# jonassibbesen/rpvg

Measured on AMD Instinct MI355X. Metric: read-pairs quantified/sec, higher is better.
Workload: dtype f64

## Files before the change

rpvg_amd/csrc/bounded_search.hip:

```cpp

#include "common.hpp"

#include <algorithm>
#include <cstdlib>
#include <map>
#include <memory>
#include <mutex>
#include <numeric>

using namespace rpvg_hip_detail;

namespace {
std::mutex g_search_gate_mutex;
const rpvg_hip_ctx * g_search_gate_owner = nullptr;
}

static bool searchLaunchesEarly() {
    static const bool early = RPVG_EXPERIMENT_ENV("RPVG_HIP_SEARCH_LAUNCH_EARLY") != nullptr;
    return early;
}

constexpr uint64_t kSearchGateRows = 1ull << 17;

static void searchGateEnter(rpvg_hip_ctx * ctx, hipStream_t stream, const uint64_t matrix_rows) {
    static const bool open_gate = RPVG_EXPERIMENT_ENV("RPVG_HIP_NO_SEARCH_GATE") != nullptr;
    ctx->search_gate_held = !open_gate && matrix_rows >= kSearchGateRows;
    if (!ctx->search_gate_held) return;
    hipEvent_t previous = nullptr;
    {
        std::lock_guard<std::mutex> lock(g_search_gate_mutex);
        if (g_search_gate_owner && g_search_gate_owner != ctx && g_search_gate_owner->device == ctx->device) {
            previous = g_search_gate_owner->search_done;
            (void) hipStreamWaitEvent(stream, previous, 0);
        }
    }
    if (previous && !searchLaunchesEarly()) (void) waitEvent(previous);
}

static void searchGateLeave(rpvg_hip_ctx * ctx, hipStream_t stream) {
    if (!ctx->search_gate_held) return;
    ctx->search_gate_held = false;
    std::lock_guard<std::mutex> lock(g_search_gate_mutex);
    (void) hipEventRecord(ctx->search_done, stream);
    g_search_gate_owner = ctx;
}

void searchGateForget(const rpvg_hip_ctx * ctx) {
    std::lock_guard<std::mutex> lock(g_search_gate_mutex);
    if (g_search_gate_owner == ctx) g_search_gate_owner = nullptr;
}

struct rpvg_hip_pair_posteriors {
    std::vector<uint64_t> pair_off;
    void * block = nullptr;
    bool block_pinned = false;
    const uint32_t * first = nullptr, * second = nullptr;
    const double * posterior = nullptr;
    ~rpvg_hip_pair_posteriors() {
        if (block && block_pinned) pinnedFree(block);
        else std::free(block);
    }
};

namespace {

constexpr uint32_t kLdsRows = 2048;
constexpr uint32_t kSmallRows = 512;
constexpr uint32_t kSmallRowLdsCols = 128;
constexpr uint32_t kRowLdsCols = 512;

__device__ __forceinline__ double waveSum(double v) { return waveSumF64(v); }

__device__ __forceinline__ double addLog(const double log_x, const double log_y) {
    return log_x > log_y ? log_x + log1p(exp(log_y - log_x)) : log_y + log1p(exp(log_x - log_y));
}


template <int kBlock, typename ValueFn>
__device__ __forceinline__ double blockLogSumExp(const uint32_t n, ValueFn value, double * scratch) {
    const double lowest = -1.7976931348623157e308;
    const int lane = threadIdx.x & 63, wave = threadIdx.x >> 6;
    double mx = lowest;
    for (uint32_t k = threadIdx.x; k < n; k += kBlock) mx = fmax(mx, value(k));
#pragma unroll
    for (int d = 32; d >= 1; d >>= 1) mx = fmax(mx, __shfl_xor(mx, d, 64));
    __syncthreads();
    if (lane == 0) scratch[wave] = mx;
    __syncthreads();
#pragma unroll
    for (int w2 = 0; w2 < kBlock / 64; ++w2) mx = fmax(mx, scratch[w2]);
    double sum = 0.0;
    for (uint32_t k = threadIdx.x; k < n; k += kBlock) {
        const double v = value(k);
        if (v > lowest) sum += exp(v - mx);
    }
    sum = waveSum(sum);
    __syncthreads();
    if (lane == 0) scratch[wave] = sum;
    __syncthreads();
    double total = 0.0;
#pragma unroll
    for (int w2 = 0; w2 < kBlock / 64; ++w2) total += scratch[w2];
    return (n == 0 || !(mx > lowest)) ? lowest : mx + log(total);
}

struct SearchArgs {
    const uint32_t * order;
    uint32_t count;
    const uint64_t * mat_val_off;
    const uint64_t * mat_row_off;
    const uint32_t * mat_fast;
    const uint32_t * mat_mid;
    const uint64_t * mat_rows;
    const uint32_t * mat_cols;
    const double * values;
    const double * rowmax;
    const double * row_count;
    const double * row_noise;
    const uint64_t * col_off;
    const uint32_t * col_count;
    const uint64_t * pair_cap_off;
    double min_log_likelihood_diff;
    uint32_t stage_rows;
    uint32_t row_lds_cols;
    double * log_freq;
    double * marginal;
    double * optimistic_raw;
    double * optimistic;
    uint32_t * col_order;
    uint32_t * out_first;
    uint32_t * out_second;
    double * out_value;
    uint32_t * out_count;
    unsigned long long * log_evals;
};

constexpr int kTileFirst = 4;

template <int kGroup>
__device__ __forceinline__ void tilePairSums(const LogTableEntry * lt, const double * lds_count, const double * lds_base, const uint32_t stride,
                                             const double * __restrict__ cnt, const double * __restrict__ nz,
                                             const double * const (&col_a)[kTileFirst], const double * __restrict__ col_b, const uint32_t staged,
                                             const uint64_t fast_end, const uint64_t mid_end, const uint64_t R, const int lane,
                                             double (&out)[kTileFirst]) {
    LogProduct pr[kTileFirst];
    double acc[kTileFirst];
#pragma unroll
    for (int t = 0; t < kTileFirst; ++t) acc[t] = 0.0;
    auto clip = [&](const uint64_t v) { return static_cast<uint32_t>(v < staged ? v : staged); };
    sumCountLogsMulti<kTileFirst, kGroup, uint32_t>(lt, lds_count, [&](const uint32_t i, double (&xs)[kTileFirst]) {
        const double x = col_b[i] / 2.0;
#pragma unroll
        for (int t = 0; t < kTileFirst; ++t) xs[t] = lds_base[t * stride + i] + x;
    }, 0u, clip(fast_end), clip(mid_end), staged, lane, pr, acc);
    if (staged < R) {
        sumCountLogsMulti<kTileFirst, kGroup, uint64_t>(lt, cnt, [&](const uint64_t i, double (&xs)[kTileFirst]) {
            const double noise = nz[i], x = col_b[i] / 2.0;
#pragma unroll
            for (int t = 0; t < kTileFirst; ++t) xs[t] = (noise + col_a[t][i] / 2.0) + x;
        }, static_cast<uint64_t>(staged), fast_end, mid_end, R, lane, pr, acc);
    }
#pragma unroll
    for (int t = 0; t < kTileFirst; ++t) out[t] = mid_end ? acc[t] + pr[t].value(lt) : acc[t];
}

template <int kBlock, int kGroup>
__global__ __launch_bounds__(kBlock) __attribute__((amdgpu_waves_per_eu(4))) void boundedSearchKernel(const SearchArgs args) {
    constexpr int kWaves = kBlock / 64;
    constexpr int kGroupsPerWave = 64 / kGroup;
    extern __shared__ __attribute__((aligned(16))) double lds_dyn[];
    double * lds_base = lds_dyn;
    double * lds_count = lds_dyn + kTileFirst * args.stage_rows;
    double * lds_rows = lds_count + args.stage_rows;
    __shared__ double lds_red[kBlock / 64];
    __shared__ unsigned long long lds_sum;
    __shared__ LogTableEntry lt[kLogTableSize];

    if (blockIdx.x >= args.count) return;
    loadLogTable(lt);
    const uint32_t m = args.order[blockIdx.x];
    const int lane = threadIdx.x & 63, wave = threadIdx.x >> 6;
    const uint64_t R = args.mat_rows[m];
    const uint32_t G = args.mat_cols[m];
    const double * M = args.values + args.mat_val_off[m];
    const double * rm = args.rowmax + args.mat_row_off[m];
    const double * cnt = args.row_count + args.mat_row_off[m];
    const double * nz = args.row_noise + args.mat_row_off[m];
    const uint64_t fast_end = args.mat_fast[m], mid_end = args.mat_mid[m];
    const uint64_t c0 = args.col_off[m];
    const uint32_t * ccount = args.col_count + c0;
    double * lf = args.log_freq + c0;
    double * marg = args.marginal + c0;
    double * opt_raw = args.optimistic_raw + c0;
    double * opt = args.optimistic + c0;
    uint32_t * ord = args.col_order + c0;
    const uint64_t p0 = args.pair_cap_off[m];
    uint32_t * out_first = args.out_first + p0;
    uint32_t * out_second = args.out_second + p0;
    double * out_value = args.out_value + p0;
    const double thr = args.min_log_likelihood_diff;
    const double lowest = -1.7976931348623157e308;
    const double log_two = log(2.0);

    if (threadIdx.x == 0) lds_sum = 0;
    __syncthreads();
    unsigned long long part = 0;
    for (uint32_t g = threadIdx.x; g < G; g += kBlock) part += ccount[g];
    if (part) atomicAdd(&lds_sum, part);
    __syncthreads();
    const double count_sum = static_cast<double>(lds_sum);
    for (uint32_t g = threadIdx.x; g < G; g += kBlock) lf[g] = log(ccount[g] / count_sum);
    __syncthreads();

    for (uint32_t g = wave; g < G; g += kWaves) {
        const double * col = M + static_cast<uint64_t>(g) * R;
        double acc1 = sumCountLogs<uint64_t>(lt, cnt, [&](const uint64_t i) { return nz[i] + col[i] / 1.0; }, 0, fast_end, mid_end, R, lane);
        double acc2 = sumCountLogs<uint64_t>(lt, cnt, [&](const uint64_t i) { return (nz[i] + col[i] / 2.0) + rm[i] / 2.0; }, 0, fast_end, mid_end, R, lane);
        acc1 = waveSum(acc1);
        acc2 = waveSum(acc2);
        if (lane == 0) {
            marg[g] = (acc1 + lf[g]) + 0.0;
            opt_raw[g] = acc2 + (lf[g] + log_two);
        }
    }
    __syncthreads();

    {
        const double sum_log = blockLogSumExp<kBlock>(G, [&](uint32_t g) { return marg[g]; }, lds_red);
        for (uint32_t g = threadIdx.x; g < G; g += kBlock) marg[g] = exp(marg[g] - sum_log);
    }
    __syncthreads();

    for (uint32_t g = threadIdx.x; g < G; g += kBlock) {
        const double pg = marg[g];
        uint32_t rank = 0;
        for (uint32_t h = 0; h < G; ++h) {
            const double ph = marg[h];
            rank += (ph > pg || (ph == pg && h > g)) ? 1u : 0u;
        }
        ord[rank] = g;
        opt[rank] = opt_raw[g];
    }
    __syncthreads();

    const bool rows_in_lds = G <= args.row_lds_cols;
    const uint32_t tile_max = rows_in_lds ? kTileFirst : 1;
    const uint32_t row_stride = rows_in_lds ? args.row_lds_cols : 0;
    double * row_ll = rows_in_lds ? lds_rows : opt_raw;
    const uint32_t stride = args.stage_rows;

    double max_ll = lowest;
    uint32_t kept = 0;
    unsigned long long pairs_evaluated = 0;
    const uint32_t staged = static_cast<uint32_t>(R < args.stage_rows ? R : args.stage_rows);
    uint32_t pos = 0;
    while (pos < G) {
        uint32_t tile_pos[kTileFirst];
        uint32_t nt = 0;
        while (pos < G && nt < tile_max) {
            if (!(opt[pos] - max_ll < thr)) tile_pos[nt++] = pos;
            ++pos;
        }
        if (nt == 0) break;
#pragma unroll
        for (int t = 1; t < kTileFirst; ++t)
            if (t >= static_cast<int>(nt)) tile_pos[t] = tile_pos[0];
        uint32_t a[kTileFirst];
        const double * col_a[kTileFirst];
#pragma unroll
        for (int t = 0; t < kTileFirst; ++t) {
            a[t] = ord[tile_pos[t]];
            col_a[t] = M + static_cast<uint64_t>(a[t]) * R;
        }
        __syncthreads();
        for (uint32_t i = threadIdx.x; i < staged; i += kBlock) {
            const double noise = nz[i];
#pragma unroll
            for (int t = 0; t < kTileFirst; ++t) lds_base[t * stride + i] = noise + col_a[t][i] / 2.0;
            lds_count[i] = cnt[i];
        }
        __syncthreads();
        for (uint32_t t = 0; t < nt; ++t) pairs_evaluated += G - tile_pos[t];
        const uint32_t j0 = tile_pos[0];
        const int sub = lane & (kGroup - 1), grp = lane / kGroup;
        for (uint32_t jw = j0 + wave * kGroupsPerWave; jw < G; jw += kWaves * kGroupsPerWave) {
            const uint32_t j = jw + grp;
            const bool valid = j < G;
            const uint32_t b = ord[valid ? j : G - 1];
            double sums[kTileFirst];
            tilePairSums<kGroup>(lt, lds_count, lds_base, stride, cnt, nz, col_a, M + static_cast<uint64_t>(b) * R, staged, fast_end, mid_end, R, sub, sums);
            const double lf_b = lf[b];
#pragma unroll
            for (int t = 0; t < kTileFirst; ++t) {
                const double total = kGroup == 64 ? waveSum(sums[t]) : rowSumF64(sums[t]);
                if (sub == 0 && valid && t < static_cast<int>(nt) && j >= tile_pos[t]) {
                    row_ll[t * row_stride + (j - tile_pos[t])] = total + ((lf[a[t]] + lf_b) + (a[t] == b ? 0.0 : log_two));
                }
            }
        }
        __syncthreads();
        for (uint32_t t = 0; t < nt; ++t) {
            if (t > 0 && opt[tile_pos[t]] - max_ll < thr) continue;
            const double * row = row_ll + t * row_stride;
            const uint32_t n = G - tile_pos[t];
            if (thr <= 0.0) {
                for (uint32_t c = 0; c < n; c += 64) {
                    const uint32_t k = c + lane;
                    const double ll = k < n ? row[k] : lowest;
                    double incl = ll;
#pragma unroll
                    for (int d = 1; d < 64; d <<= 1) {
                        const double up = __shfl_up(incl, d, 64);
                        if (lane >= d) incl = fmax(incl, up);
                    }
                    double before = __shfl_up(incl, 1, 64);
                    before = lane == 0 ? max_ll : fmax(max_ll, before);
                    const bool keep = k < n && !(ll - before < thr);
                    const unsigned long long ballot = __ballot(keep);
                    if (keep && wave == 0) {
                        const uint32_t slot = kept + __popcll(ballot & ((1ull << lane) - 1ull));
                        out_first[slot] = a[t];
                        out_second[slot] = ord[tile_pos[t] + k];
                        out_value[slot] = ll;
                    }
                    kept += __popcll(ballot);
                    max_ll = fmax(max_ll, __shfl(incl, 63, 64));
                }
            } else {
                for (uint32_t k = 0; k < n; ++k) {
                    const double ll = row[k];
                    if (!(ll - max_ll < thr)) {
                        max_ll = fmax(max_ll, ll);
                        if (threadIdx.x == 0) {
                            out_first[kept] = a[t];
                            out_second[kept] = ord[tile_pos[t] + k];
                            out_value[kept] = ll;
                        }
                        ++kept;
                    }
                }
            }
        }
    }

    __syncthreads();
    if (threadIdx.x == 0) {
        args.out_count[m] = kept;
        atomicAdd(args.log_evals, (2ull * G + pairs_evaluated) * R);
    }
    {
        auto kept_value = [&](uint32_t k) { const double ll = out_value[k]; return (ll - max_ll < thr) ? lowest : ll; };
        const double sum_log = blockLogSumExp<kBlock>(kept, kept_value, lds_red);
        for (uint32_t k = threadIdx.x; k < kept; k += kBlock) out_value[k] = exp(kept_value(k) - sum_log);
    }
}



constexpr uint32_t kChunkRows = 1024;
constexpr int kTileA = 4;

struct TableWork {
    const uint32_t * item_matrix;
    const uint32_t * item_col;
    const uint32_t * item_chunk;
    uint32_t count;
    const uint64_t * mat_val_off;
    const uint64_t * mat_row_off;
    const uint32_t * mat_fast;
    const uint32_t * mat_mid;
    const uint64_t * mat_rows;
    const uint32_t * mat_cols;
    const double * values;
    const double * rowmax;
    const double * row_count;
    const double * row_noise;
    const uint64_t * big_col_part_off;
    const uint64_t * big_pair_part_off;
    double * part_marginal;
    double * part_optimistic;
    double * part_pair;
    unsigned long long * log_evals;
};

__global__ __launch_bounds__(256) void pairTableKernel(const TableWork w) {
    __shared__ double lds_base[kTileA][kChunkRows];
    __shared__ double lds_count[kChunkRows];
    __shared__ LogTableEntry lt[kLogTableSize];
    const uint32_t per_xcd = (w.count + 7) / 8;
    const uint32_t item = (blockIdx.x % 8) * per_xcd + blockIdx.x / 8;
    if (item >= w.count) return;
    loadLogTable(lt);
    const uint32_t m = w.item_matrix[item], a0 = w.item_col[item], chunk = w.item_chunk[item];
    const int lane = threadIdx.x & 63, wave = threadIdx.x >> 6;
    const uint64_t R = w.mat_rows[m];
    const uint32_t G = w.mat_cols[m];
    const uint32_t ta = (G - a0) < kTileA ? (G - a0) : kTileA;
    const uint64_t r_begin = static_cast<uint64_t>(chunk) * kChunkRows;
    const uint32_t n = static_cast<uint32_t>((R - r_begin) < kChunkRows ? (R - r_begin) : kChunkRows);
    const double * M = w.values + w.mat_val_off[m] + r_begin;
    const double * cnt = w.row_count + w.mat_row_off[m] + r_begin;
    const double * nz = w.row_noise + w.mat_row_off[m] + r_begin;
    auto local = [&](const uint64_t end_row) { return end_row <= r_begin ? 0u : (end_row - r_begin < n ? static_cast<uint32_t>(end_row - r_begin) : n); };
    const uint32_t nf = local(w.mat_fast[m]), nm = local(w.mat_mid[m]);

    for (uint32_t i = threadIdx.x; i < n; i += 256) {
        const double noise = nz[i];
        lds_count[i] = cnt[i];
#pragma unroll
        for (int t = 0; t < kTileA; ++t) {
            const uint32_t a = a0 + (t < static_cast<int>(ta) ? t : 0);
            lds_base[t][i] = noise + M[static_cast<uint64_t>(a) * R + i] / 2.0;
        }
    }
    __syncthreads();
    const uint32_t num_tasks = ta + (G - a0);
    for (uint32_t task = wave; task < num_tasks; task += 4) {
        if (task < ta) {
            const uint32_t a = a0 + task;
            const double * col_a = M + static_cast<uint64_t>(a) * R;
            const double acc = waveSum(sumCountLogs<uint32_t>(lt, lds_count, [&](const uint32_t i) { return nz[i] + col_a[i] / 1.0; }, 0u, nf, nm, n, lane));
            if (lane == 0) w.part_marginal[w.big_col_part_off[m] + static_cast<uint64_t>(chunk) * G + a] = acc;
        } else {
            const uint32_t b = a0 + (task - ta);
            const double * col_b = M + static_cast<uint64_t>(b) * R;
            double acc[kTileA];
            LogProduct pr[kTileA];
#pragma unroll
            for (int t = 0; t < kTileA; ++t) acc[t] = 0.0;
            sumCountLogsMulti<kTileA, 64, uint32_t>(lt, lds_count, [&](const uint32_t i, double (&xs)[kTileA]) {
                const double x = col_b[i] / 2.0;
#pragma unroll
                for (int t = 0; t < kTileA; ++t) xs[t] = lds_base[t][i] + x;
            }, 0u, nf, nm, n, lane, pr, acc);
            if (nm) {
#pragma unroll
                for (int t = 0; t < kTileA; ++t) acc[t] += pr[t].value(lt);
            }
#pragma unroll
            for (int t = 0; t < kTileA; ++t) {
                const double total = waveSum(acc[t]);
                if (lane == 0 && t < static_cast<int>(ta) && a0 + t <= b) {
                    w.part_pair[w.big_pair_part_off[m] + (static_cast<uint64_t>(chunk) * G + (a0 + t)) * G + b] = total;
                }
            }
        }
    }
    if (threadIdx.x == 0) atomicAdd(w.log_evals, static_cast<unsigned long long>(ta + (G - a0) * kTileA) * n);
}


constexpr uint32_t kTileBlock = 256;
constexpr uint32_t kTileLdsDoubles = 6 * 1024;
constexpr uint32_t kTileMaxColumns = 1024;

__host__ __device__ inline uint32_t tileColumns(const uint32_t G) { return (G + 3) / 4; }
__host__ __device__ inline uint32_t tileCount(const uint32_t G) { return tileColumns(G) * (tileColumns(G) + 1) / 2; }
__host__ __device__ inline uint32_t tileSlices(const uint32_t G) { return tileCount(G) <= kTileBlock ? kTileBlock / tileCount(G) : 1u; }
__host__ __device__ inline uint32_t marginalSlices(const uint32_t G) { return kTileBlock / tileColumns(G); }

struct PairTileWork {
    const uint32_t * item_matrix;
    const uint32_t * item_chunk;
    const uint32_t * item_tiles;
    uint32_t chunk_rows;
    uint32_t count;
    const uint64_t * mat_val_off;
    const uint64_t * mat_row_off;
    const uint32_t * mat_fast;
    const uint32_t * mat_mid;
    const uint64_t * mat_rows;
    const uint32_t * mat_cols;
    const double * values;
    const double * row_count;
    const double * row_noise;
    const uint64_t * col_part_off;
    const uint64_t * pair_part_off;
    double * part_marginal;
    double * part_pair;
    unsigned long long * log_evals;
#ifdef RPVG_HIP_EXPERIMENTS
    uint32_t debug_skip;
#endif
};

#ifdef RPVG_HIP_EXPERIMENTS
#define RPVG_PAIR_DEBUG_SKIP(w) ((w).debug_skip)
#else
#define RPVG_PAIR_DEBUG_SKIP(w) 0u
#endif

constexpr uint32_t kTile2BufferDoubles = 3 * 1024;

__host__ __device__ inline uint32_t tileRowOfTile(const uint32_t t, const uint32_t T) {
    uint32_t lo = 0, hi = T - 1;
    while (lo < hi) {
        const uint32_t mid = (lo + hi + 1) >> 1;
        if (mid * T - mid * (mid - 1) / 2 <= t) lo = mid; else hi = mid - 1;
    }
    return lo;
}

__device__ __forceinline__ void ldsDirectLoad16(const double * from, double * lds_wave_base) {
    __builtin_amdgcn_global_load_lds((const __attribute__((address_space(1))) void *)from, (__attribute__((address_space(3))) void *)lds_wave_base, 16, 0, 0);
}

template <uint32_t kSubRows>
__device__ __forceinline__ void ldsReadRow(const uint32_t noise_at, const uint32_t u_at, const uint32_t v_at, double & noise, double (&u)[4], double (&v)[4]) {
    asm volatile("ds_read_b64 %0, %9\n\t"
                 "ds_read_b64 %1, %10\n\t"
                 "ds_read_b64 %2, %10 offset:%12\n\t"
                 "ds_read_b64 %3, %10 offset:%13\n\t"
                 "ds_read_b64 %4, %10 offset:%14\n\t"
                 "ds_read_b64 %5, %11\n\t"
                 "ds_read_b64 %6, %11 offset:%12\n\t"
                 "ds_read_b64 %7, %11 offset:%13\n\t"
                 "ds_read_b64 %8, %11 offset:%14"
                 : "=&v"(noise), "=&v"(u[0]), "=&v"(u[1]), "=&v"(u[2]), "=&v"(u[3]), "=&v"(v[0]), "=&v"(v[1]), "=&v"(v[2]), "=&v"(v[3])
                 : "v"(noise_at), "v"(u_at), "v"(v_at), "i"(kSubRows * 8), "i"(kSubRows * 16), "i"(kSubRows * 24));
}

__device__ __forceinline__ void ldsRowLanded(double & noise, double (&u)[4], double (&v)[4]) {
    asm volatile("s_waitcnt lgkmcnt(0)" : "+v"(noise), "+v"(u[0]), "+v"(u[1]), "+v"(u[2]), "+v"(u[3]), "+v"(v[0]), "+v"(v[1]), "+v"(v[2]), "+v"(v[3]));
}

__device__ __forceinline__ uint32_t ldsByteAddress(const double * const p) {
    return static_cast<uint32_t>(reinterpret_cast<uintptr_t>(p));
}

__host__ __device__ inline uint32_t tileSubRows(const uint32_t ncols) {
    const uint32_t fit = (kTile2BufferDoubles - ncols / 2) / (ncols + 2);
    return fit >= 126 ? 126u : fit >= 94 ? 94u : fit >= 46 ? 46u : fit >= 30 ? 30u : fit >= 14 ? 14u : fit >= 6 ? 6u : 2u;
}

template <uint32_t kSubRows>
__device__ __forceinline__ void pairTile2Item(const PairTileWork & w, double * const tile_lds, const LogTableEntry * const lt, const uint32_t m, const uint32_t chunk,
                                              const uint32_t t0, const uint32_t tcount, const uint32_t c_lo, const uint32_t ncols) {
    const uint64_t R = w.mat_rows[m];
    const uint32_t G = w.mat_cols[m];
    const uint32_t T = tileColumns(G);
    const uint32_t S = kTileBlock / tcount;
    constexpr uint32_t sub_rows = kSubRows;
    const uint32_t lanes_per_column = sub_rows / 2, columns_per_load = lanes_per_column <= 16 ? 4u : lanes_per_column <= 32 ? 2u : 1u;
    auto columnOffset = [&](const uint32_t c) { return static_cast<size_t>(c) * sub_rows + (c / 4) * 2; };
    const uint64_t r_begin = static_cast<uint64_t>(chunk) * w.chunk_rows;
    const uint32_t n = static_cast<uint32_t>((R - r_begin) < w.chunk_rows ? (R - r_begin) : w.chunk_rows);
    const double * M = w.values + w.mat_val_off[m] + r_begin;
    const double * cnt = w.row_count + w.mat_row_off[m] + r_begin;
    const double * nz = w.row_noise + w.mat_row_off[m] + r_begin;
    auto local = [&](const uint64_t end_row) { return end_row <= r_begin ? 0u : (end_row - r_begin < n ? static_cast<uint32_t>(end_row - r_begin) : n); };
    const uint32_t nf = local(w.mat_fast[m]), nm = local(w.mat_mid[m]);
    const uint32_t lane = threadIdx.x & 63u, wave = threadIdx.x >> 6;

    const uint32_t buffer_doubles = (ncols + 2) * sub_rows + ncols / 2;
    auto stage = [&](const uint32_t s0, const uint32_t ns, double * const buffer) {
        if (RPVG_PAIR_DEBUG_SKIP(w) & 16u) return;
        const uint32_t pairs = (ns + 1) / 2;
        const uint32_t col_in_load = lane / lanes_per_column, pair = lane % lanes_per_column;
        const bool lane_loads = col_in_load < columns_per_load && pair < pairs;
        for (uint32_t c0 = wave * columns_per_load; c0 < ncols; c0 += 4 * columns_per_load) {
            const uint32_t c = c0 + col_in_load;
            if (lane_loads && c < ncols) {
                const uint32_t column = c_lo + c < G ? c_lo + c : G - 1;
                ldsDirectLoad16(M + static_cast<uint64_t>(column) * R + s0 + 2 * pair, buffer + columnOffset(c0));
            }
        }
        if (wave < 2 && lane < pairs) {
            ldsDirectLoad16((wave == 0 ? nz : cnt) + s0 + 2 * lane, buffer + columnOffset(ncols) + wave * sub_rows);
        }
    };

    const uint32_t t = t0 + threadIdx.x % tcount, slice = threadIdx.x / tcount;
    const bool active = slice < S;
    const uint32_t ta = tileRowOfTile(t, T);
    const uint32_t tb = ta + (t - (ta * T - ta * (ta > 0 ? ta - 1 : 0) / 2));
    const uint32_t SM = marginalSlices(G);
    const uint32_t tc = threadIdx.x % T, marg_slice = threadIdx.x / T;
    const bool with_marginals = t0 == 0 && marg_slice < SM && !(RPVG_PAIR_DEBUG_SKIP(w) & 8u);

    LogProduct pr[4][4], prm[4];
    double acc[4][4], accm[4];
#pragma unroll
    for (int i = 0; i < 4; ++i) {
        accm[i] = 0.0;
#pragma unroll
        for (int j = 0; j < 4; ++j) acc[i][j] = 0.0;
    }
    uint32_t since_fold = 0, since_fold_m = 0;
    int doubled = 0;
    auto foldPairs = [&]() {
#pragma unroll
        for (int i = 0; i < 4; ++i) {
#pragma unroll
            for (int j = 0; j < 4; ++j) pr[i][j].fold();
        }
        since_fold = 0;
    };
    auto foldMarginals = [&]() {
#pragma unroll
        for (int i = 0; i < 4; ++i) prm[i].fold();
        since_fold_m = 0;
    };

    const uint32_t blocks = (n + sub_rows - 1) / sub_rows;
    if (RPVG_PAIR_DEBUG_SKIP(w) & 64u) return;
    if (RPVG_PAIR_DEBUG_SKIP(w) & 16u) {
        for (uint32_t i = threadIdx.x; i < 2 * kTile2BufferDoubles; i += kTileBlock) tile_lds[i] = 0.25;
    }
    stage(0, n < sub_rows ? n : sub_rows, tile_lds);
    for (uint32_t blk = 0; blk < blocks; ++blk) {
        const uint32_t s0 = blk * sub_rows;
        const uint32_t ns = (n - s0) < sub_rows ? (n - s0) : sub_rows;
        double * const H = tile_lds + static_cast<size_t>(blk & 1u) * buffer_doubles;
        asm volatile("s_waitcnt vmcnt(0)" ::: "memory");
        __syncthreads();
        if (blk + 1 < blocks) {
            const uint32_t s1 = s0 + sub_rows;
            stage(s1, (n - s1) < sub_rows ? (n - s1) : sub_rows, tile_lds + static_cast<size_t>((blk + 1) & 1u) * buffer_doubles);
        }
        const double * const lds_noise = H + columnOffset(ncols);
        const double * const lds_count = lds_noise + sub_rows;
        const uint32_t f1 = nf <= s0 ? 0u : ((nf - s0) < ns ? (nf - s0) : ns);
        const uint32_t m1 = nm <= s0 ? 0u : ((nm - s0) < ns ? (nm - s0) : ns);
        if (active) {
            const double * const ua = H + columnOffset(4 * ta - c_lo), * const vb = H + columnOffset(4 * tb - c_lo);
            uint32_t r = (RPVG_PAIR_DEBUG_SKIP(w) & 1u) ? f1 : slice;
            {
                uint32_t noise_at = ldsByteAddress(lds_noise + r), u_at = ldsByteAddress(ua + r), v_at = ldsByteAddress(vb + r);
                for (; r < f1; r += S, noise_at += 8 * S, u_at += 8 * S, v_at += 8 * S) {
                    double noise, u[4], v[4];
                    ldsReadRow<kSubRows>(noise_at, u_at, v_at, noise, u, v);
                    ldsRowLanded(noise, u, v);
                    const double un[4] = {fma(2.0, noise, u[0]), fma(2.0, noise, u[1]), fma(2.0, noise, u[2]), fma(2.0, noise, u[3])};
#pragma unroll
                    for (int i = 0; i < 4; ++i) {
#pragma unroll
                        for (int j = 0; j < 4; ++j) pr[i][j].mul(un[i] + v[j]);
                    }
                    doubled += 1;
                    if (++since_fold == kFoldFactors) foldPairs();
                }
            }
            for (r = (RPVG_PAIR_DEBUG_SKIP(w) & 2u) ? m1 : f1 + (slice + S - f1 % S) % S; r < m1; r += S) {
                double noise, u[4], v[4];
                ldsReadRow<kSubRows>(ldsByteAddress(lds_noise + r), ldsByteAddress(ua + r), ldsByteAddress(vb + r), noise, u, v);
                ldsRowLanded(noise, u, v);
                const uint32_t c = static_cast<uint32_t>(lds_count[r]);
                const double un[4] = {fma(2.0, noise, u[0]), fma(2.0, noise, u[1]), fma(2.0, noise, u[2]), fma(2.0, noise, u[3])};
                if (since_fold + c > kFoldFactors) foldPairs();
                since_fold += c;
                doubled += static_cast<int>(c);
                double x[4][4];
#pragma unroll
                for (int i = 0; i < 4; ++i) {
#pragma unroll
                    for (int j = 0; j < 4; ++j) x[i][j] = un[i] + v[j];
                }
                for (uint32_t k = 0; k < c; ++k) {
#pragma unroll
                    for (int i = 0; i < 4; ++i) {
#pragma unroll
                        for (int j = 0; j < 4; ++j) pr[i][j].mul(x[i][j]);
                    }
                }
            }
            for (r = (RPVG_PAIR_DEBUG_SKIP(w) & 4u) ? ns : m1 + (slice + S - m1 % S) % S; r < ns; r += S) {
                const double noise = lds_noise[r], c = lds_count[r];
                const double un[4] = {fma(2.0, noise, ua[r]), fma(2.0, noise, ua[sub_rows + r]), fma(2.0, noise, ua[2 * sub_rows + r]), fma(2.0, noise, ua[3 * sub_rows + r])};
                const double v[4] = {vb[r], vb[sub_rows + r], vb[2 * sub_rows + r], vb[3 * sub_rows + r]};
#pragma unroll
                for (int i = 0; i < 4; ++i) {
#pragma unroll
                    for (int j = 0; j < 4; ++j) acc[i][j] = fma(c, logPositive(0.5 * (un[i] + v[j]), lt), acc[i][j]);
                }
            }
        }
        if (with_marginals) {
            const double * const ua = H + columnOffset(4 * tc);
            for (uint32_t r = marg_slice; r < ns; r += SM) {
                const double noise = lds_noise[r];
                const double x[4] = {ua[r] + noise, ua[sub_rows + r] + noise, ua[2 * sub_rows + r] + noise, ua[3 * sub_rows + r] + noise};
                if (r < f1) {
#pragma unroll
                    for (int i = 0; i < 4; ++i) prm[i].mul(x[i]);
                    if (++since_fold_m == kFoldFactors) foldMarginals();
                } else if (r < m1) {
                    const uint32_t c = static_cast<uint32_t>(lds_count[r]);
                    if (since_fold_m + c > kFoldFactors) foldMarginals();
                    since_fold_m += c;
                    for (uint32_t k = 0; k < c; ++k) {
#pragma unroll
                        for (int i = 0; i < 4; ++i) prm[i].mul(x[i]);
                    }
                } else {
                    const double c = lds_count[r];
#pragma unroll
                    for (int i = 0; i < 4; ++i) accm[i] = fma(c, logPositive(x[i], lt), accm[i]);
                }
            }
        }
    }
    if (RPVG_PAIR_DEBUG_SKIP(w) & 32u) return;
    double * const out_pairs = w.part_pair + w.pair_part_off[m] + static_cast<uint64_t>(chunk) * G * G;
    double * const out_columns = w.part_marginal + w.col_part_off[m] + static_cast<uint64_t>(chunk) * G;
    double * const sums = tile_lds;
    double * const column_sums = tile_lds;
    if (S > 1) __syncthreads();
    if (active) {
#pragma unroll
        for (int i = 0; i < 4; ++i) {
#pragma unroll
            for (int j = 0; j < 4; ++j) {
                const uint32_t a = 4 * ta + i, b = 4 * tb + j;
                pr[i][j].fold();
                pr[i][j].e -= doubled;
                const double total = acc[i][j] + pr[i][j].value(lt);
                if (S > 1) sums[(slice * tcount + (t - t0)) * 16 + i * 4 + j] = total;
                else if (a <= b && b < G) out_pairs[static_cast<uint64_t>(a) * G + b] = total;
            }
        }
    }
    if (S > 1) {
        __syncthreads();
        for (uint32_t e = threadIdx.x; e < tcount * 16; e += kTileBlock) {
            double total = 0.0;
            for (uint32_t sl = 0; sl < S; ++sl) total += sums[sl * tcount * 16 + e];
            const uint32_t te = t0 + e / 16, i = (e % 16) / 4, j = e % 4;
            const uint32_t row = tileRowOfTile(te, T);
            const uint32_t a = 4 * row + i, b = 4 * (row + (te - (row * T - row * (row > 0 ? row - 1 : 0) / 2))) + j;
            if (a <= b && b < G) out_pairs[static_cast<uint64_t>(a) * G + b] = total;
        }
    }
    if (t0 == 0 && !(RPVG_PAIR_DEBUG_SKIP(w) & 8u)) {
        if (SM > 1) __syncthreads();
        if (with_marginals) {
#pragma unroll
            for (int i = 0; i < 4; ++i) {
                const uint32_t a = 4 * tc + i;
                const double total = accm[i] + prm[i].value(lt);
                if (SM > 1) column_sums[(marg_slice * T + tc) * 4 + i] = total;
                else if (a < G) out_columns[a] = total;
            }
        }
        if (SM > 1) {
            __syncthreads();
            for (uint32_t e = threadIdx.x; e < T * 4; e += kTileBlock) {
                double total = 0.0;
                for (uint32_t sl = 0; sl < SM; ++sl) total += column_sums[sl * T * 4 + e];
                if (e < G) out_columns[e] = total;
            }
        }
    }
    if (threadIdx.x == 0 && t0 == 0) atomicAdd(w.log_evals, static_cast<unsigned long long>(static_cast<uint64_t>(G) * (G + 1) / 2 + G) * n);
}

__global__ __launch_bounds__(kTileBlock) __attribute__((amdgpu_waves_per_eu(3))) void pairTile2Kernel(const PairTileWork w) {
    extern __shared__ __attribute__((aligned(16))) double tile_lds[];
    __shared__ LogTableEntry lt[kLogTableSize];
    const uint32_t item = blockIdx.x;
    if (item >= w.count) return;
    const uint32_t m = w.item_matrix[item], chunk = w.item_chunk[item];
    const uint32_t t0 = w.item_tiles[item] & 0xffffu, tcount = (w.item_tiles[item] >> 16) + 1;
    if (RPVG_PAIR_DEBUG_SKIP(w) & 128u) return;
    loadLogTable(lt);
    const uint32_t T = tileColumns(w.mat_cols[m]);
    const uint32_t c_lo = 4 * tileRowOfTile(t0, T), ncols = 4 * T - c_lo;
    switch (tileSubRows(ncols)) {
        case 126: pairTile2Item<126>(w, tile_lds, lt, m, chunk, t0, tcount, c_lo, ncols); break;
        case 94: pairTile2Item<94>(w, tile_lds, lt, m, chunk, t0, tcount, c_lo, ncols); break;
        case 46: pairTile2Item<46>(w, tile_lds, lt, m, chunk, t0, tcount, c_lo, ncols); break;
        case 30: pairTile2Item<30>(w, tile_lds, lt, m, chunk, t0, tcount, c_lo, ncols); break;
        case 14: pairTile2Item<14>(w, tile_lds, lt, m, chunk, t0, tcount, c_lo, ncols); break;
        case 6: pairTile2Item<6>(w, tile_lds, lt, m, chunk, t0, tcount, c_lo, ncols); break;
        default: pairTile2Item<2>(w, tile_lds, lt, m, chunk, t0, tcount, c_lo, ncols); break;
    }
}

inline void planTileRanges(const uint32_t tiles, std::vector<std::pair<uint32_t, uint32_t> > * ranges) {
    uint32_t t0 = 0, left = tiles;
    while (left > 0) {
        if (left >= kTileBlock) {
            ranges->emplace_back(t0, kTileBlock);
            t0 += kTileBlock;
            left -= kTileBlock;
            continue;
        }
        const uint32_t slices = kTileBlock / left;
        const uint32_t more = kTileBlock / (slices + 1), rest = left - more;
        const double one = 1.0 / slices, two = 1.0 / (slices + 1) + 1.0 / (kTileBlock / rest);
        if (two < 0.9 * one) {
            ranges->emplace_back(t0, more);
            t0 += more;
            left = rest;
        } else {
            ranges->emplace_back(t0, left);
            left = 0;
        }
    }
}

struct ResolveArgs {
    const uint32_t * big_matrix;
    uint32_t chunk_rows;
    uint32_t count;
    const uint64_t * mat_rows;
    const uint32_t * mat_cols;
    const uint64_t * col_off;
    const uint32_t * col_count;
    const uint64_t * pair_cap_off;
    const uint64_t * big_col_part_off;
    const uint64_t * big_pair_part_off;
    const double * part_marginal;
    const double * part_optimistic;
    const double * part_pair;
    double min_log_likelihood_diff;
    double * log_freq;
    double * marginal;
    uint32_t * col_order;
    double * seq_value;
    uint32_t * out_first;
    uint32_t * out_second;
    double * out_value;
    uint32_t * out_count;
};

__device__ __forceinline__ uint64_t sequenceRowStart(const uint32_t pos, const uint32_t G) {
    return static_cast<uint64_t>(pos) * G - (static_cast<uint64_t>(pos) * (pos > 0 ? pos - 1 : 0)) / 2;
}

__device__ __forceinline__ uint32_t sequenceRow(const uint64_t slot, const uint32_t G) {
    uint32_t lo = 0, hi = G - 1;
    while (lo < hi) {
        const uint32_t mid = (lo + hi + 1) >> 1;
        if (sequenceRowStart(mid, G) <= slot) lo = mid; else hi = mid - 1;
    }
    return lo;
}

__global__ __launch_bounds__(256) void resolveTableKernel(const ResolveArgs args) {
    constexpr int kBlock = 256;
    __shared__ double lds_red[kBlock / 64];
    __shared__ uint32_t lds_cnt[kBlock / 64];
    __shared__ unsigned long long lds_sum;
    if (blockIdx.x >= args.count) return;
    const uint32_t m = args.big_matrix[blockIdx.x];
    const int lane = threadIdx.x & 63, wave = threadIdx.x >> 6;
    const uint64_t R = args.mat_rows[m];
    const uint32_t G = args.mat_cols[m];
    const uint32_t chunks = static_cast<uint32_t>((R + args.chunk_rows - 1) / args.chunk_rows);
    const uint64_t c0 = args.col_off[m];
    const uint32_t * ccount = args.col_count + c0;
    double * lf = args.log_freq + c0;
    double * marg = args.marginal + c0;
    uint32_t * ord = args.col_order + c0;
    const double * pm = args.part_marginal + args.big_col_part_off[m];
    const double * pp = args.part_pair + args.big_pair_part_off[m];
    const uint64_t p0 = args.pair_cap_off[m];
    double * seq = args.seq_value + p0;
    uint32_t * out_first = args.out_first + p0;
    uint32_t * out_second = args.out_second + p0;
    double * out_value = args.out_value + p0;
    const double thr = args.min_log_likelihood_diff;
    const double lowest = -1.7976931348623157e308;
    const double log_two = log(2.0);

    if (threadIdx.x == 0) lds_sum = 0;
    __syncthreads();
    unsigned long long part = 0;
    for (uint32_t g = threadIdx.x; g < G; g += kBlock) part += ccount[g];
    if (part) atomicAdd(&lds_sum, part);
    __syncthreads();
    const double count_sum = static_cast<double>(lds_sum);
    for (uint32_t g = threadIdx.x; g < G; g += kBlock) {
        const double f = log(ccount[g] / count_sum);
        lf[g] = f;
        double acc = 0.0;
        for (uint32_t c = 0; c < chunks; ++c) acc += pm[static_cast<uint64_t>(c) * G + g];
        marg[g] = (acc + f) + 0.0;
    }
    __syncthreads();
    {
        const double sum_log = blockLogSumExp<kBlock>(G, [&](uint32_t g) { return marg[g]; }, lds_red);
        for (uint32_t g = threadIdx.x; g < G; g += kBlock) marg[g] = exp(marg[g] - sum_log);
    }
    __syncthreads();
    for (uint32_t g = threadIdx.x; g < G; g += kBlock) {
        const double pg = marg[g];
        uint32_t rank = 0;
        for (uint32_t h = 0; h < G; ++h) {
            const double ph = marg[h];
            rank += (ph > pg || (ph == pg && h > g)) ? 1u : 0u;
        }
        ord[rank] = g;
    }
    __syncthreads();

    const uint64_t S = static_cast<uint64_t>(G) * (G + 1) / 2;
    for (uint64_t slot = threadIdx.x; slot < S; slot += kBlock) {
        const uint32_t pos = sequenceRow(slot, G);
        const uint32_t j = pos + static_cast<uint32_t>(slot - sequenceRowStart(pos, G));
        const uint32_t a = ord[pos], b = ord[j];
        const uint32_t lo = a < b ? a : b, hi = a < b ? b : a;
        double acc = 0.0;
        for (uint32_t c = 0; c < chunks; ++c) acc += pp[(static_cast<uint64_t>(c) * G + lo) * G + hi];
        seq[slot] = acc + ((lf[a] + lf[b]) + (a == b ? 0.0 : log_two));
    }
    __syncthreads();

    double carry_max = lowest;
    uint32_t kept = 0;
    for (uint64_t base = 0; base < S; base += kBlock) {
        const uint64_t s = base + threadIdx.x;
        const double v = s < S ? seq[s] : lowest;
        double inc = v;
#pragma unroll
        for (int d = 1; d < 64; d <<= 1) {
            const double t = __shfl_up(inc, d, 64);
            if (lane >= d) inc = fmax(inc, t);
        }
        if (lane == 63) lds_red[wave] = inc;
        __syncthreads();
        double before = carry_max, total = carry_max;
#pragma unroll
        for (int w2 = 0; w2 < kBlock / 64; ++w2) {
            if (w2 < wave) before = fmax(before, lds_red[w2]);
            total = fmax(total, lds_red[w2]);
        }
        double excl = __shfl_up(inc, 1, 64);
        if (lane == 0) excl = lowest;
        excl = fmax(excl, before);
        const bool keep = (s < S) && !(v - excl < thr);
        const unsigned long long ballot = __ballot(keep);
        const uint32_t in_wave = __popcll(ballot & ((1ull << lane) - 1ull));
        if (lane == 0) lds_cnt[wave] = __popcll(ballot);
        __syncthreads();
        uint32_t off = kept, tot = 0;
#pragma unroll
        for (int w2 = 0; w2 < kBlock / 64; ++w2) {
            if (w2 < wave) off += lds_cnt[w2];
            tot += lds_cnt[w2];
        }
        if (keep) {
            const uint32_t pos = sequenceRow(s, G);
            const uint32_t j = pos + static_cast<uint32_t>(s - sequenceRowStart(pos, G));
            out_first[off + in_wave] = ord[pos];
            out_second[off + in_wave] = ord[j];
            out_value[off + in_wave] = v;
        }
        kept += tot;
        carry_max = total;
        __syncthreads();
    }
    const double max_ll = carry_max;

    __syncthreads();
    if (threadIdx.x == 0) args.out_count[m] = kept;
    {
        auto kept_value = [&](uint32_t k) { const double ll = out_value[k]; return (ll - max_ll < thr) ? lowest : ll; };
        const double sum_log = blockLogSumExp<kBlock>(kept, kept_value, lds_red);
        for (uint32_t k = threadIdx.x; k < kept; k += kBlock) out_value[k] = exp(kept_value(k) - sum_log);
    }
}

__global__ void __launch_bounds__(1024) pairOffsetsKernel(const uint32_t num_matrices, const uint32_t * __restrict__ counts,
                                                          uint64_t * __restrict__ pair_off, const uint32_t * __restrict__ build_error,
                                                          uint32_t * __restrict__ build_error_out, uint32_t * __restrict__ tail_copy,
                                                          const uint32_t tail_words) {
    __shared__ uint64_t sums[1024];
    const uint32_t per = (num_matrices + 1023) / 1024;
    const uint32_t lo = min(num_matrices, threadIdx.x * per), hi = min(num_matrices, lo + per);
    uint64_t mine = 0;
    for (uint32_t m = lo; m < hi; ++m) mine += counts[m];
    sums[threadIdx.x] = mine;
    __syncthreads();
    for (uint32_t step = 1; step < 1024; step <<= 1) {
        const uint64_t add = threadIdx.x >= step ? sums[threadIdx.x - step] : 0;
        __syncthreads();
        sums[threadIdx.x] += add;
        __syncthreads();
    }
    uint64_t run = sums[threadIdx.x] - mine;
    for (uint32_t m = lo; m < hi; ++m) {
        pair_off[m] = run;
        run += counts[m];
    }
    if (threadIdx.x == 1023) pair_off[num_matrices] = sums[1023];
    if (threadIdx.x == 0 && build_error) *build_error_out = *build_error;
    __syncthreads();
    for (uint32_t i = threadIdx.x; i < tail_words; i += blockDim.x) tail_copy[i] = counts[i];
}

__global__ void compactPairsBlockKernel(const uint32_t num_matrices, const uint64_t * __restrict__ pair_cap_off,
                                        const uint64_t * __restrict__ pair_off, const uint32_t * __restrict__ in_first,
                                        const uint32_t * __restrict__ in_second, const double * __restrict__ in_value,
                                        unsigned char * __restrict__ block) {
    const uint32_t m = blockIdx.x;
    if (m >= num_matrices) return;
    const uint64_t total = pair_off[num_matrices];
    double * out_value = reinterpret_cast<double *>(block);
    uint32_t * out_first = reinterpret_cast<uint32_t *>(block + total * sizeof(double));
    uint32_t * out_second = out_first + total;
    const uint64_t src = pair_cap_off[m], dst = pair_off[m], n = pair_off[m + 1] - pair_off[m];
    for (uint64_t k = threadIdx.x; k < n; k += blockDim.x) {
        out_first[dst + k] = in_first[src + k];
        out_second[dst + k] = in_second[src + k];
        out_value[dst + k] = in_value[src + k];
    }
}

}

namespace rpvg_hip_detail {

int queuePairSearch(rpvg_hip_ctx * ctx, const rpvg_hip_groups * groups, const uint32_t * column_counts, const double min_rel_likelihood,
                    PairSearchWork & w) {
    std::unique_ptr<HostScope> scope(new HostScope("bounded search: host order + work items"));
    const uint32_t M = groups->num_matrices;
    w.M = M;
    std::vector<uint64_t> & col_off = w.col_off, & pair_cap_off = w.pair_cap_off;
    col_off.assign(M + 1, 0);
    pair_cap_off.assign(M + 1, 0);
    for (uint32_t m = 0; m < M; ++m) {
        const uint64_t G = groups->h_num_cols[m];
        col_off[m + 1] = col_off[m] + G;
        pair_cap_off[m + 1] = pair_cap_off[m] + G * (G + 1) / 2;
    }
    if (!column_counts && M > 0 && !groups->d_column_counts) {
        setError("rpvg_hip_bounded_pair_posteriors: column_counts is NULL");
        return RPVG_HIP_ERR_INVALID;
    }
    for (uint64_t c = 0; column_counts && c < col_off[M]; ++c) {
        if (column_counts[c] == 0) {
            setError("rpvg_hip_bounded_pair_posteriors: column %llu has a zero count", static_cast<unsigned long long>(c));
            return RPVG_HIP_ERR_INVALID;
        }
    }
    std::vector<uint32_t> & order = w.order;
    order.assign(M, 0);
    std::iota(order.begin(), order.end(), 0);
    std::sort(order.begin(), order.end(), [&](uint32_t x, uint32_t y) {
        const double wx = static_cast<double>(groups->h_num_rows[x]) * groups->h_num_cols[x] * groups->h_num_cols[x];
        const double wy = static_cast<double>(groups->h_num_rows[y]) * groups->h_num_cols[y] * groups->h_num_cols[y];
        return wx != wy ? wx > wy : x < y;
    });

    const uint64_t table_budget = 1ull << 28;
    double table_min_work = 65536.0;
    if (const char * env = std::getenv("RPVG_HIP_TABLE_MIN_WORK")) table_min_work = std::atof(env);
    if (min_rel_likelihood > 1) table_min_work = 1e300;
    const char * tiles_env = std::getenv("RPVG_HIP_PAIR_TILES");
    const int tiles_wanted = tiles_env ? std::atoi(tiles_env) : 2;
// ... 490 lines not shown
```

Before: 2.416 billion.

## Software-pipeline LDS row reads and specialise product-only blocks without log path

Double-buffers the LDS row loads in the doubled-factor loop so the next row's ds_reads are in flight while the current row's products run. A partial s_waitcnt lets the older loads land first. Splits the block loop into product-only blocks and log-row blocks via a compile-time flag, so early blocks skip the log-evaluation code paths. Changes the slice-reduction LDS layout so each active thread reduces its own tile entries, replacing the strided cross-thread reduction. These add register pressure and code size, and the fold check now runs every two rows instead of every row.

```diff
diff --git a/rpvg_amd/csrc/bounded_search.hip b/rpvg_amd/csrc/bounded_search.hip
--- a/rpvg_amd/csrc/bounded_search.hip
+++ b/rpvg_amd/csrc/bounded_search.hip
@@ -7,6 +7,7 @@
 #include <memory>
 #include <mutex>
 #include <numeric>
+#include <type_traits>
 
 using namespace rpvg_hip_detail;
 
@@ -524,6 +525,10 @@
     asm volatile("s_waitcnt lgkmcnt(0)" : "+v"(noise), "+v"(u[0]), "+v"(u[1]), "+v"(u[2]), "+v"(u[3]), "+v"(v[0]), "+v"(v[1]), "+v"(v[2]), "+v"(v[3]));
 }
 
+__device__ __forceinline__ void ldsRowLandedBeforeNext(double & noise, double (&u)[4], double (&v)[4]) {
+    asm volatile("s_waitcnt lgkmcnt(9)" : "+v"(noise), "+v"(u[0]), "+v"(u[1]), "+v"(u[2]), "+v"(u[3]), "+v"(v[0]), "+v"(v[1]), "+v"(v[2]), "+v"(v[3]));
+}
+
 __device__ __forceinline__ uint32_t ldsByteAddress(const double * const p) {
     return static_cast<uint32_t>(reinterpret_cast<uintptr_t>(p));
 }
@@ -608,7 +613,8 @@
         for (uint32_t i = threadIdx.x; i < 2 * kTile2BufferDoubles; i += kTileBlock) tile_lds[i] = 0.25;
     }
     stage(0, n < sub_rows ? n : sub_rows, tile_lds);
-    for (uint32_t blk = 0; blk < blocks; ++blk) {
+    auto block = [&](const uint32_t blk, auto log_rows) {
+        constexpr bool kLogRows = decltype(log_rows)::value;
         const uint32_t s0 = blk * sub_rows;
         const uint32_t ns = (n - s0) < sub_rows ? (n - s0) : sub_rows;
         double * const H = tile_lds + static_cast<size_t>(blk & 1u) * buffer_doubles;
@@ -625,21 +631,45 @@
         if (active) {
             const double * const ua = H + columnOffset(4 * ta - c_lo), * const vb = H + columnOffset(4 * tb - c_lo);
             uint32_t r = (RPVG_PAIR_DEBUG_SKIP(w) & 1u) ? f1 : slice;
-            {
+            if (r < f1) {
                 uint32_t noise_at = ldsByteAddress(lds_noise + r), u_at = ldsByteAddress(ua + r), v_at = ldsByteAddress(vb + r);
-                for (; r < f1; r += S, noise_at += 8 * S, u_at += 8 * S, v_at += 8 * S) {
-                    double noise, u[4], v[4];
-                    ldsReadRow<kSubRows>(noise_at, u_at, v_at, noise, u, v);
-                    ldsRowLanded(noise, u, v);
+                auto factors = [&](const double noise, const double (&u)[4], const double (&v)[4]) {
                     const double un[4] = {fma(2.0, noise, u[0]), fma(2.0, noise, u[1]), fma(2.0, noise, u[2]), fma(2.0, noise, u[3])};
 #pragma unroll
                     for (int i = 0; i < 4; ++i) {
 #pragma unroll
                         for (int j = 0; j < 4; ++j) pr[i][j].mul(un[i] + v[j]);
                     }
+                };
+                double noise0, u0[4], v0[4], noise1, u1[4], v1[4];
+                ldsReadRow<kSubRows>(noise_at, u_at, v_at, noise0, u0, v0);
+                for (; r + 2 * S < f1; r += 2 * S) {
+                    ldsReadRow<kSubRows>(noise_at + 8 * S, u_at + 8 * S, v_at + 8 * S, noise1, u1, v1);
+                    ldsRowLandedBeforeNext(noise0, u0, v0);
+                    factors(noise0, u0, v0);
+                    noise_at += 16 * S, u_at += 16 * S, v_at += 16 * S;
+                    ldsReadRow<kSubRows>(noise_at, u_at, v_at, noise0, u0, v0);
+                    ldsRowLandedBeforeNext(noise1, u1, v1);
+                    factors(noise1, u1, v1);
+                    doubled += 2;
+                    since_fold += 2;
+                    if (since_fold >= kFoldFactors) foldPairs();
+                }
+                if (r + S < f1) {
+                    ldsReadRow<kSubRows>(noise_at + 8 * S, u_at + 8 * S, v_at + 8 * S, noise1, u1, v1);
+                    ldsRowLandedBeforeNext(noise0, u0, v0);
+                    factors(noise0, u0, v0);
+                    ldsRowLanded(noise1, u1, v1);
+                    factors(noise1, u1, v1);
+                    doubled += 2;
+                    since_fold += 2;
+                } else {
+                    ldsRowLanded(noise0, u0, v0);
+                    factors(noise0, u0, v0);
                     doubled += 1;
-                    if (++since_fold == kFoldFactors) foldPairs();
+                    since_fold += 1;
                 }
+                if (since_fold >= kFoldFactors) foldPairs();
             }
             for (r = (RPVG_PAIR_DEBUG_SKIP(w) & 2u) ? m1 : f1 + (slice + S - f1 % S) % S; r < m1; r += S) {
                 double noise, u[4], v[4];
@@ -664,6 +694,7 @@
                     }
                 }
             }
+            if constexpr (kLogRows)
             for (r = (RPVG_PAIR_DEBUG_SKIP(w) & 4u) ? ns : m1 + (slice + S - m1 % S) % S; r < ns; r += S) {
                 const double noise = lds_noise[r], c = lds_count[r];
                 const double un[4] = {fma(2.0, noise, ua[r]), fma(2.0, noise, ua[sub_rows + r]), fma(2.0, noise, ua[2 * sub_rows + r]), fma(2.0, noise, ua[3 * sub_rows + r])};
@@ -692,14 +723,17 @@
 #pragma unroll
                         for (int i = 0; i < 4; ++i) prm[i].mul(x[i]);
                     }
-                } else {
+                } else if constexpr (kLogRows) {
                     const double c = lds_count[r];
 #pragma unroll
                     for (int i = 0; i < 4; ++i) accm[i] = fma(c, logPositive(x[i], lt), accm[i]);
                 }
             }
         }
-    }
+    };
+    const uint32_t product_blocks = nm >= n ? blocks : nm / sub_rows;
+    for (uint32_t blk = 0; blk < product_blocks; ++blk) block(blk, std::false_type());
+    for (uint32_t blk = product_blocks; blk < blocks; ++blk) block(blk, std::true_type());
     if (RPVG_PAIR_DEBUG_SKIP(w) & 32u) return;
     double * const out_pairs = w.part_pair + w.pair_part_off[m] + static_cast<uint64_t>(chunk) * G * G;
     double * const out_columns = w.part_marginal + w.col_part_off[m] + static_cast<uint64_t>(chunk) * G;
@@ -715,20 +749,20 @@
                 pr[i][j].fold();
                 pr[i][j].e -= doubled;
                 const double total = acc[i][j] + pr[i][j].value(lt);
-                if (S > 1) sums[(slice * tcount + (t - t0)) * 16 + i * 4 + j] = total;
+                if (S > 1) sums[(slice * 16 + i * 4 + j) * tcount + (t - t0)] = total;
                 else if (a <= b && b < G) out_pairs[static_cast<uint64_t>(a) * G + b] = total;
             }
         }
     }
     if (S > 1) {
         __syncthreads();
-        for (uint32_t e = threadIdx.x; e < tcount * 16; e += kTileBlock) {
-            double total = 0.0;
-            for (uint32_t sl = 0; sl < S; ++sl) total += sums[sl * tcount * 16 + e];
-            const uint32_t te = t0 + e / 16, i = (e % 16) / 4, j = e % 4;
-            const uint32_t row = tileRowOfTile(te, T);
-            const uint32_t a = 4 * row + i, b = 4 * (row + (te - (row * T - row * (row > 0 ? row - 1 : 0) / 2))) + j;
-            if (a <= b && b < G) out_pairs[static_cast<uint64_t>(a) * G + b] = total;
+        if (active) {
+            for (uint32_t k = slice; k < 16; k += S) {
+                double total = 0.0;
+                for (uint32_t sl = 0; sl < S; ++sl) total += sums[(sl * 16 + k) * tcount + (t - t0)];
+                const uint32_t a = 4 * ta + k / 4, b = 4 * tb + k % 4;
+                if (a <= b && b < G) out_pairs[static_cast<uint64_t>(a) * G + b] = total;
+            }
         }
     }
     if (t0 == 0 && !(RPVG_PAIR_DEBUG_SKIP(w) & 8u)) {
@@ -738,7 +772,7 @@
             for (int i = 0; i < 4; ++i) {
                 const uint32_t a = 4 * tc + i;
                 const double total = accm[i] + prm[i].value(lt);
-                if (SM > 1) column_sums[(marg_slice * T + tc) * 4 + i] = total;
+                if (SM > 1) column_sums[(marg_slice * 4 + i) * T + tc] = total;
                 else if (a < G) out_columns[a] = total;
             }
         }
@@ -746,7 +780,7 @@
             __syncthreads();
             for (uint32_t e = threadIdx.x; e < T * 4; e += kTileBlock) {
                 double total = 0.0;
-                for (uint32_t sl = 0; sl < SM; ++sl) total += column_sums[sl * T * 4 + e];
+                for (uint32_t sl = 0; sl < SM; ++sl) total += column_sums[(sl * 4 + e % 4) * T + e / 4];
                 if (e < G) out_columns[e] = total;
             }
         }
```

New measurement: 2.411 billion (median of 3 runs). Within noise of the previous version (-0.2%).
